# VinAIResearch/GeoFormer

Measured on NVIDIA B200. Metric: geodesic maps/sec, higher is better.
Workload: dtype f32

## Files before the change

### geoformer_b200/_capi.py

```python
import ctypes
import os
import threading

import torch

_HERE = os.path.dirname(os.path.abspath(__file__))
LIB_PATH = os.environ.get("GF_LIB") or os.path.join(_HERE, "libgeoformer_b200.so")

_lib = None
_lock = threading.Lock()

c_int, c_float, c_size_t, c_void_p, c_int64 = ctypes.c_int, ctypes.c_float, ctypes.c_size_t, ctypes.c_void_p, ctypes.c_int64

_P = c_void_p
SIGNATURES = {
    "gf_last_error": (ctypes.c_char_p, []),
    "gf_version": (c_int, []),
    "gf_launch_count": (c_int64, []),
    "gf_reset_launch_count": (None, []),
    "gf_set_stage_events": (c_int, [_P, c_int]),
    "gf_event_create": (c_void_p, []),
    "gf_event_destroy": (None, [_P]),
    "gf_event_elapsed_ms": (c_float, [_P, _P]),
    "gf_fps_workspace_bytes": (c_size_t, [c_int, c_int, c_int]),
    "gf_furthest_point_sampling": (c_int, [_P, c_int, c_int, c_int, _P, _P, c_size_t, _P]),
    "gf_gather_points": (c_int, [_P, _P, c_int, c_int, c_int, c_int, _P, _P]),
    "gf_gather_points_grad": (c_int, [_P, _P, c_int, c_int, c_int, c_int, _P, _P]),
    "gf_ball_query": (c_int, [_P, _P, c_int, c_int, c_int, c_float, c_int, _P, _P]),
    "gf_group_points": (c_int, [_P, _P, c_int, c_int, c_int, c_int, c_int, _P, _P]),
    "gf_group_points_grad": (c_int, [_P, _P, c_int, c_int, c_int, c_int, c_int, _P, _P]),
    "gf_three_nn": (c_int, [_P, _P, c_int, c_int, c_int, _P, _P, _P]),
    "gf_three_interpolate": (c_int, [_P, _P, _P, c_int, c_int, c_int, c_int, _P, _P]),
    "gf_three_interpolate_grad": (c_int, [_P, _P, _P, c_int, c_int, c_int, c_int, _P, _P]),
    "gf_knn_workspace_bytes": (c_size_t, [c_int, c_int, c_int, c_int]),
    "gf_knn": (c_int, [_P, c_int, _P, c_int, c_int, c_int, _P, _P, _P, c_int, _P, c_size_t, _P]),
    "gf_geodesic_workspace_bytes": (c_size_t, [c_int, c_int, c_int]),
    "gf_geodesic": (c_int, [_P, _P, c_int, c_int, c_int, _P, c_int, c_float, c_int, _P, _P, _P, _P, c_size_t, _P]),
    "gf_bias_workspace_bytes": (c_size_t, [c_int, c_int]),
    "gf_bias_decoder": (c_int, [_P, _P, _P, _P, _P, c_int, c_int, c_int, _P, _P, c_size_t, _P]),
    "gf_bias_decoder_fourier": (c_int, [_P, _P, _P, _P, _P, c_int, c_int, c_int, _P, c_int, c_int, _P, _P, _P, _P,
                                        c_size_t, _P]),
    "gf_bias_mask_head": (c_int, [_P, _P, _P, c_int, c_int, _P, _P, _P, c_size_t, _P]),
    "gf_rel_cross_attention_workspace_bytes": (c_size_t, [c_int, c_int, c_int]),
    "gf_rel_cross_attention": (c_int, [_P, _P, _P, c_int, c_int, c_int, _P, _P, _P, _P, _P, _P, _P, _P, _P, _P, c_size_t, _P]),
    "gf_rel_cross_attention_fused": (c_int, [_P, _P, _P, _P, _P, _P, _P, _P, c_int, _P, _P, c_int, c_int, c_int,
                                             _P, _P, _P, _P, _P, _P, _P, _P, _P, _P, c_size_t, _P]),
    "gf_rel_cross_attention_save": (c_int, [_P, _P, _P, c_int, c_int, c_int] + [_P] * 12 + [c_size_t, _P]),
    "gf_rel_cross_attention_fused_save": (c_int, [_P] * 8 + [c_int, _P, _P, c_int, c_int, c_int] + [_P] * 12
                                          + [c_size_t, _P]),
    "gf_rel_cross_attention_backward_workspace_bytes": (c_size_t, [c_int, c_int, c_int]),
    "gf_rel_cross_attention_backward": (c_int, [_P, _P, _P, c_int, c_int, c_int] + [_P] * 24 + [c_size_t, _P]),
    "gf_rel_cross_attention_fused_backward": (c_int, [_P] * 8 + [c_int, _P, _P, c_int, c_int, c_int] + [_P] * 23
                                              + [c_size_t, _P]),
    "gf_mask_head_workspace_bytes": (c_size_t, [c_int, c_int]),
    "gf_mask_head_logits": (c_int, [_P] * 9 + [c_int, c_int, c_int, _P, _P, c_size_t, _P]),
    "gf_mask_head_backward_workspace_bytes": (c_size_t, [c_int, c_int]),
    "gf_mask_head_logits_backward": (c_int, [_P] * 9 + [c_int, c_int, c_int] + [_P] * 7 + [c_size_t, _P]),
    "gf_group_mlp_pool": (c_int, [_P, _P, _P, _P, c_int, c_int, c_int, c_int, c_int, c_float, c_int, c_int, c_int, _P, _P,
# ... 116 lines not shown
```

### geoformer_b200/csrc/gf_guidance.cu

```cuda
#include <stdlib.h>

#include "gf_geodesic.cuh"
#include "gf_knn.cuh"

namespace gf {

constexpr int LANES = 4;
struct ForkJoin {
  cudaStream_t fps[LANES] = {}, knn[LANES] = {};
  cudaEvent_t fork = nullptr, join_fps[LANES] = {}, join_knn[LANES] = {};
  cudaStream_t aux = nullptr;
  cudaEvent_t join = nullptr;
};

static int get_fork_join(cudaStream_t user, ForkJoin **out, int lanes_needed = 1) {
  constexpr int SLOTS = 16;
  struct Entry {
    int dev;
    cudaStream_t user;
    ForkJoin fj;
    bool used;
  };
  static thread_local Entry pool[SLOTS];
  static thread_local int next_victim = 0;
// ... 124 lines not shown

extern "C" int gf_guidance_seeded(const float *xyz, int N, const int *seeds, int Q, int k, float radius, int max_step,
                                  float *geo, float *knn_dist, int32_t *knn_idx32, int64_t *stats, float *row_max,
                                  void *workspace, size_t workspace_bytes, void *stream) {
  return guidance_impl(xyz, N, Q, k, radius, max_step, const_cast<int *>(seeds), 1, geo, knn_dist, knn_idx32, stats,
                       workspace, workspace_bytes, stream, nullptr, 0, row_max);
}

extern "C" int gf_guidance_shard(const float *xyz, int N, int Q, int q0, int q1, int k, float radius, int max_step,
                                 int *seeds, float *geo_block, int64_t *stats, float *row_max_block, void *workspace,
                                 size_t workspace_bytes, void *stream) {
  return guidance_impl(xyz, N, Q, k, radius, max_step, seeds, 0, geo_block, nullptr, nullptr, stats, workspace,
                       workspace_bytes, stream, nullptr, 0, row_max_block, q0, q1);
}

extern "C" int gf_guidance_seeded_scatter(const float *xyz, int N, const int *seeds, int Q, int k, float radius,
                                          int max_step, float *geo, float *const *peer_geo, int n_peers,
                                          int64_t *stats, void *workspace, size_t workspace_bytes, void *stream) {
  return guidance_impl(xyz, N, Q, k, radius, max_step, const_cast<int *>(seeds), 1, geo, nullptr, nullptr, stats,
                       workspace, workspace_bytes, stream, peer_geo, n_peers);
}

namespace gf {
struct BatchPlan {
  size_t per_scene[GEO_BATCH_MAX * 4];
  size_t scratch, scratch_bytes, stats, total;
};
static int plan_batch_guidance(const int *Ns, int B, int Q, int k, BatchPlan *p, size_t *fps_b, size_t *knn_b,
                               size_t *edge_b) {
  size_t off = 0;
  int maxN = 1;
  for (int b = 0; b < B; ++b) {
    const int N = Ns[b];
    fps_b[b] = align256(gf_fps_workspace_bytes(1, N, Q));
    knn_b[b] = align256(knn_grid_workspace_bytes(N));
    edge_b[b] = align256(geodesic_workspace_bytes(N, k, 1));
    p->per_scene[b * 3 + 0] = off, off += fps_b[b];
    p->per_scene[b * 3 + 1] = off, off += knn_b[b];
    p->per_scene[b * 3 + 2] = off, off += edge_b[b];
    maxN = N > maxN ? N : maxN;
  }
  p->scratch = off;
  p->scratch_bytes = align256(geodesic_batch_scratch_bytes(maxN, (long long)Q * B));
  off += p->scratch_bytes;
  p->stats = off;
  off += align256(16 * (size_t)B);
  p->total = off + 1024;
  return maxN;
}
}

extern "C" size_t gf_guidance_batch_workspace_bytes(const int *Ns, int B, int Q, int k) {
  if (!Ns || B <= 0 || B > GEO_BATCH_MAX || Q <= 0 || k <= 0) return 0;
  for (int b = 0; b < B; ++b)
    if (Ns[b] <= 0) return 0;
  BatchPlan p;
  size_t f[GEO_BATCH_MAX], n[GEO_BATCH_MAX], e[GEO_BATCH_MAX];
  plan_batch_guidance(Ns, B, Q, k, &p, f, n, e);
  return p.total;
}

extern "C" int gf_guidance_batch(const float *const *xyz, const int *Ns, int B, int Q, int k, float radius,
                                 int max_step, int *const *seeds, int seeds_given, float *const *geo,
                                 float *const *row_max, int64_t *stats, void *workspace, size_t workspace_bytes,
// ... 2 lines not shown
  GF_CHECK_ARG(B >= 1 && B <= GEO_BATCH_MAX, "guidance_batch: B=%d outside [1,%d]", B, GEO_BATCH_MAX);
  GF_CHECK_ARG(Q >= 1, "guidance_batch: need Q >= 1");
  GF_CHECK_ARG(k >= 1 && k <= KNN_MAX_K, "guidance_batch: k=%d outside [1,%d]", k, KNN_MAX_K);
  for (int b = 0; b < B; ++b) {
    GF_CHECK_ARG(Ns[b] >= 1 && xyz[b] && seeds[b] && geo[b], "guidance_batch: scene %d: empty or null", b);
    GF_CHECK_ARG(geodesic_edge_format(Ns[b]) == 1,
                 "guidance_batch: scene %d has %d points, beyond the on-chip bitmaps of the batched kernel "
                 "(use gf_guidance per scene)", b, Ns[b]);
  }
  BatchPlan p;
  size_t fps_b[GEO_BATCH_MAX], knn_b[GEO_BATCH_MAX], edge_b[GEO_BATCH_MAX];
  plan_batch_guidance(Ns, B, Q, k, &p, fps_b, knn_b, edge_b);
  if (workspace == nullptr || workspace_bytes < p.total) {
    set_error("guidance_batch: workspace too small (%zu bytes given, %zu needed)", workspace_bytes, p.total);
    return GF_ERR_WORKSPACE;
  }
  cudaStream_t st = (cudaStream_t)stream;
  char *w = (char *)workspace;
  ForkJoin *fj = nullptr;
  const int lanes = B < LANES ? B : LANES;
  int rc = get_fork_join(st, &fj, lanes);
  if (rc) return rc;
  stage_mark(ST_BEGIN, st);
  GF_CUDA(cudaEventRecord(fj->fork, st));
  for (int l = 0; l < lanes; ++l) {
    if (!seeds_given) GF_CUDA(cudaStreamWaitEvent(fj->fps[l], fj->fork, 0));
    if (l > 0) GF_CUDA(cudaStreamWaitEvent(fj->knn[l], fj->fork, 0));
  }
  GeoSceneDesc desc[GEO_BATCH_MAX];
  int64_t *d_stats = stats ? (int64_t *)(w + p.stats) : nullptr;
  if (d_stats) GF_CUDA(cudaMemsetAsync(d_stats, 0, 16 * (size_t)B, st));
  if (!seeds_given)
    for (int b = 0; b < B; ++b) {
      rc = gf_furthest_point_sampling(xyz[b], 1, Ns[b], Q, seeds[b], w + p.per_scene[b * 3 + 0], fps_b[b],
                                      fj->fps[b % lanes]);
      if (rc) return rc;
    }
  for (int b = 0; b < B; ++b) {
    const int l = b % lanes;
    cudaStream_t ks = l == 0 ? st : fj->knn[l];
    KnnGridBuffers gb;
    rc = knn_grid_build(xyz[b], Ns[b], k, w + p.per_scene[b * 3 + 1], knn_b[b], ks, &gb);
    if (rc) return rc;
    KnnEdgeOut eo;
    eo.radius = radius;
    int enc = 0;
    rc = geodesic_edge_buffers(w + p.per_scene[b * 3 + 2], edge_b[b], Ns[b], k, 1, &eo.tgt, &eo.len, &eo.slot_bits,
                               &enc);
    if (rc) return rc;
    eo.rank = gb.rank;
    rc = knn_grid_query(gb, nullptr, Ns[b], k, 1, nullptr, nullptr, nullptr, ks, &eo);
    if (rc) return rc;
    desc[b].tgt = eo.tgt, desc[b].len = eo.len, desc[b].seeds = seeds[b], desc[b].geo = geo[b];
    desc[b].rank = gb.rank, desc[b].order = gb.order;
    desc[b].row_max = row_max ? row_max[b] : nullptr;
    desc[b].stats = d_stats ? d_stats + 2 * b : nullptr;
    desc[b].N = Ns[b], desc[b].Q = Q;
  }
  for (int l = 0; l < lanes; ++l) {
    if (!seeds_given) {
      GF_CUDA(cudaEventRecord(fj->join_fps[l], fj->fps[l]));
      GF_CUDA(cudaStreamWaitEvent(st, fj->join_fps[l], 0));
    }
    if (l > 0) {
      GF_CUDA(cudaEventRecord(fj->join_knn[l], fj->knn[l]));
      GF_CUDA(cudaStreamWaitEvent(st, fj->join_knn[l], 0));
    }
  }
  stage_mark(ST_KNN_DONE, st);
  rc = geodesic_batch_launch(desc, B, k, max_step, w + p.scratch, p.scratch_bytes, st);
  if (rc) return rc;
  if (stats) GF_CUDA(cudaMemcpyAsync(stats, d_stats, 16 * (size_t)B, cudaMemcpyDeviceToDevice, st));
  return GF_OK;
}

extern "C" size_t gf_guidance_host_workspace_bytes(int N, int Q, int k) {
  if (N <= 0 || Q <= 0 || k <= 0) return 0;
  return plan_guidance(N, Q, k).total + align256(sizeof(float) * (size_t)N * 3) + align256(sizeof(int) * (size_t)Q) +
         align256(sizeof(float) * (size_t)Q * N) + 1024;
}

extern "C" int gf_guidance_host(const float *xyz_host, int N, int Q, int k, float radius, int max_step,
                                int *seeds_host, float *geo_host, void *workspace, size_t workspace_bytes,
                                void *stream) {
  GF_CHECK_ARG(N >= 1 && Q >= 1, "guidance_host: need N >= 1 and Q >= 1");
  GF_CHECK_ARG(xyz_host && seeds_host && geo_host, "guidance_host: null host pointer");
  size_t need = gf_guidance_host_workspace_bytes(N, Q, k);
// ... 117 lines not shown
```

### geoformer_b200/csrc/gf_knn.cu

```cuda
#include "gf_knn.cuh"

namespace gf {

constexpr int KNN_MAX_CELLS = 1 << 22;
constexpr int KNN_PASS0_CELLS = 1 << 18;
constexpr int KNN_SCAN_BLOCKS = 512;
constexpr int KNN_MAX_DIM = 1024;

struct KnnGrid {
  float ox, oy, oz;
  float h, inv_h;
  float slack;
  int dx, dy, dz, ncells;
  uint32_t mm[6];
  unsigned long long sum_sq;
  unsigned done[2];
  unsigned pad_[2];
};
struct KnnCtl {
  KnnGrid g;
  unsigned long long scan_state[KNN_SCAN_BLOCKS];
};

__device__ void knn_plan(KnnGrid *g, int N, int pass, float tau, int cap) {
// ... 45 lines not shown
  __shared__ bool s_last;
  __threadfence();
  __syncthreads();
  if (threadIdx.x == 0) {
    const unsigned t = atomicAdd(counter, 1u);
    s_last = t == gridDim.x - 1;
    __threadfence();
  }
  __syncthreads();
  return s_last;
}

__device__ __forceinline__ int cell_coord(float v, float o, float inv_h, int dim) {
  float f = floorf((v - o) * inv_h);
  int c = (f >= 0.f) ? (f < (float)dim ? (int)f : dim - 1) : 0;
  return c;
}
__device__ __forceinline__ int cell_of(const KnnGrid &g, float x, float y, float z) {
  int cx = cell_coord(x, g.ox, g.inv_h, g.dx), cy = cell_coord(y, g.oy, g.inv_h, g.dy),
      cz = cell_coord(z, g.oz, g.inv_h, g.dz);
  return (cz * g.dy + cy) * g.dx + cx;
}

__global__ void __launch_bounds__(256) knn_bbox_kernel(const float *__restrict__ xyz, int N, KnnGrid *g, float tau,
                                                       int cap_coarse, int4 *__restrict__ zero_a, int n4_a,
                                                       int4 *__restrict__ zero_b, int n4_b) {
  const int gtid = blockIdx.x * blockDim.x + threadIdx.x, gsz = gridDim.x * blockDim.x;
  const int4 z4 = make_int4(0, 0, 0, 0);
  for (int i = gtid; i < n4_a; i += gsz) zero_a[i] = z4;
  for (int i = gtid; i < n4_b; i += gsz) zero_b[i] = z4;
  uint32_t lo[3] = {0u, 0u, 0u}, hi[3] = {0u, 0u, 0u};
  for (int i = gtid; i < N; i += gsz) {
#pragma unroll
    for (int a = 0; a < 3; ++a) {
      float v = __ldg(xyz + (size_t)i * 3 + a);
      if (v == v && fabsf(v) <= 3.0e38f) {
        uint32_t o = f2ord(v);
        lo[a] = max(lo[a], ~o);
        hi[a] = max(hi[a], o);
      }
    }
  }
#pragma unroll
  for (int a = 0; a < 3; ++a) {
    uint32_t l = __reduce_max_sync(0xffffffffu, lo[a]);
    uint32_t h = __reduce_max_sync(0xffffffffu, hi[a]);
    if ((threadIdx.x & 31) == 0) {
      if (l) atomicMax(&g->mm[a], l);
      if (h) atomicMax(&g->mm[3 + a], h);
    }
  }
  if (last_block_done(&g->done[0]) && threadIdx.x == 0) knn_plan(g, N, 0, tau, cap_coarse);
}

__global__ void __launch_bounds__(256) knn_count_kernel(const float *__restrict__ xyz, int N, KnnGrid *gp,
                                                        int *__restrict__ cell_count, int *__restrict__ cell_id,
                                                        int *__restrict__ slot_in_cell, float tau, int cap_fine) {
  const KnnGrid g = *gp;
  unsigned long long acc = 0;
  for (int i = blockIdx.x * blockDim.x + threadIdx.x; i < N; i += gridDim.x * blockDim.x) {
    float x = __ldg(xyz + (size_t)i * 3), y = __ldg(xyz + (size_t)i * 3 + 1), z = __ldg(xyz + (size_t)i * 3 + 2);
    int c = cell_of(g, x, y, z);
    int s = atomicAdd(cell_count + c, 1);
    if (cell_id) {
      cell_id[i] = c;
      slot_in_cell[i] = s;
    } else {
      acc += 2ull * (unsigned)s + 1ull;
    }
  }
  if (cell_id) return;
  for (int o = 16; o; o >>= 1) acc += __shfl_xor_sync(0xffffffffu, acc, o);
  if ((threadIdx.x & 31) == 0 && acc) atomicAdd(&gp->sum_sq, acc);
  if (last_block_done(&gp->done[1]) && threadIdx.x == 0) knn_plan(gp, N, 1, tau, cap_fine);
}

__global__ void __launch_bounds__(256) knn_scan_kernel(KnnCtl *ctl, const int *__restrict__ cnt,
                                                       int *__restrict__ start, int N) {
  const int n = ctl->g.ncells;
  const int chunk = (((n + KNN_SCAN_BLOCKS - 1) / KNN_SCAN_BLOCKS) + 3) & ~3;
  const int b0 = min(n, (int)blockIdx.x * chunk), b1 = min(n, b0 + chunk);
  __shared__ int ws[8];
  __shared__ int carry;
  const int lane = threadIdx.x & 31, warp = threadIdx.x >> 5;
  int acc = 0;
  for (int i = b0 + threadIdx.x; i < b1; i += 256) acc += cnt[i];
  for (int o = 16; o; o >>= 1) acc += __shfl_xor_sync(0xffffffffu, acc, o);
  if (lane == 0) ws[warp] = acc;
  __syncthreads();
  volatile unsigned long long *state = ctl->scan_state;
  if (threadIdx.x == 0) {
    int t = 0;
    for (int w = 0; w < 8; ++w) t += ws[w];
    state[blockIdx.x] = (1ull << 63) | (unsigned long long)(unsigned)t;
  }
  int pre = 0;
  for (int j = threadIdx.x; j < (int)blockIdx.x; j += 256) {
    unsigned long long v;
    while (!((v = state[j]) >> 63)) __nanosleep(20);
    pre += (int)(unsigned)(v & 0xffffffffull);
  }
  for (int o = 16; o; o >>= 1) pre += __shfl_xor_sync(0xffffffffu, pre, o);
  __syncthreads();
// ... 13 lines not shown
    for (int e = 0; e < 4; ++e) c[e] = (i0 + e < b1) ? cnt[i0 + e] : 0;
    int tsum = c[0] + c[1] + c[2] + c[3];
    int inc = tsum;
    for (int o = 1; o < 32; o <<= 1) {
      int t = __shfl_up_sync(0xffffffffu, inc, o);
      if (lane >= o) inc += t;
    }
    if (lane == 31) ws[warp] = inc;
    __syncthreads();
    int woff = 0;
    for (int w = 0; w < warp; ++w) woff += ws[w];
    int excl = carry + woff + inc - tsum;
#pragma unroll
    for (int e = 0; e < 4; ++e) {
      if (i0 + e < b1) start[i0 + e] = excl;
      excl += c[e];
    }
    __syncthreads();
    if (threadIdx.x == 255) carry = excl;
    __syncthreads();
  }
}

__global__ void knn_scatter_kernel(const float *__restrict__ xyz, int N, const int *__restrict__ cell_id,
                                   const int *__restrict__ slot_in_cell, const int *__restrict__ start,
                                   float4 *__restrict__ sorted, int *__restrict__ order, int *__restrict__ rank) {
  for (int i = blockIdx.x * blockDim.x + threadIdx.x; i < N; i += gridDim.x * blockDim.x) {
    int pos = start[cell_id[i]] + slot_in_cell[i];
    float x = __ldg(xyz + (size_t)i * 3), y = __ldg(xyz + (size_t)i * 3 + 1), z = __ldg(xyz + (size_t)i * 3 + 2);
    sorted[pos] = make_float4(x, y, z, __int_as_float(i));
    order[pos] = i;
    rank[i] = pos;
  }
}

template <int KT>
struct TopK {
  unsigned long long key[KT];
  __device__ __forceinline__ void init(int k) {
#pragma unroll
    for (int i = 0; i < KT; ++i) key[i] = (i < KT - k) ? 0ull : ~0ull;
  }
  __device__ __forceinline__ void offer(float d2, int index) {
    unsigned long long kk = ((unsigned long long)__float_as_uint(d2) << 32) | (unsigned)index;
    if (kk < key[KT - 1]) {
      bool below = true;
#pragma unroll
      for (int i = KT - 1; i > 0; --i) {
        const bool below_prev = kk < key[i - 1];
        key[i] = below_prev ? key[i - 1] : (below ? kk : key[i]);
// ... 55 lines not shown
        len[e] = ok ? d : 0.f;
      }
    }
    for (int e = k - 1 > 0 ? k - 1 : 0; e < KP; ++e) tgt[e] = none, len[e] = 0.f;
  }
  __device__ __forceinline__ void store(int k, bool do_sqrt, float *__restrict__ dist, long long *__restrict__ i64,
                                        int *__restrict__ i32) const {
#pragma unroll
    for (int i = 0; i < KT; ++i) {
      int j = i - (KT - k);
      if (j >= 0) {
        unsigned long long kk = key[i];
        bool missing = kk == ~0ull;
        float d2 = missing ? __int_as_float(0x7f800000) : __uint_as_float((unsigned)(kk >> 32));
        int id = missing ? -1 : (int)(unsigned)(kk & 0xffffffffu);
        if (dist) dist[j] = do_sqrt ? sqrtf(d2) : d2;
        if (i64) i64[j] = (long long)id;
        if (i32) i32[j] = id;
      }
    }
  }
};

constexpr int KNN_NB = 32;
constexpr int KNN_MIN_BLOCKS = 7;
template <int KT>
__global__ void __launch_bounds__(128, KT <= 16 ? KNN_MIN_BLOCKS : 1)
    knn_grid_query_kernel(const KnnGrid *__restrict__ gp, const float4 *__restrict__ sorted,
                          const int *__restrict__ start, const float *__restrict__ queries, int nq, int k,
                          int do_sqrt, float *__restrict__ dist, long long *__restrict__ idx64,
                          int *__restrict__ idx32, const KnnEdgeOut eo) {
  constexpr int LIST = KT + 16;
  __shared__ unsigned short hist[KNN_NB][128];
  __shared__ int list[LIST][128];
  const KnnGrid g = *gp;
  const int tid = threadIdx.x;
  const int s = blockIdx.x * blockDim.x + tid;
  if (s >= nq) return;
  if (eo.tgt && s == 0) {
    const int none = eo.rank ? (int)((((unsigned)nq >> 5) << 7) | ((unsigned)nq & 31u)) : nq;
    for (int e = 0; e < (1 << eo.slot_bits); ++e)
      eo.tgt[((size_t)nq << eo.slot_bits) + e] = none, eo.len[((size_t)nq << eo.slot_bits) + e] = 0.f;
  }
  float qx, qy, qz;
  int row;
  if (queries == nullptr) {
    float4 me = sorted[s];
    qx = me.x, qy = me.y, qz = me.z;
    row = __float_as_int(me.w);
  } else {
    qx = __ldg(queries + (size_t)s * 3), qy = __ldg(queries + (size_t)s * 3 + 1), qz = __ldg(queries + (size_t)s * 3 + 2);
    row = s;
  }
  const int cx = cell_coord(qx, g.ox, g.inv_h, g.dx), cy = cell_coord(qy, g.oy, g.inv_h, g.dy),
            cz = cell_coord(qz, g.oz, g.inv_h, g.dz);
  TopK<KT> top;
  top.init(k);
  auto offer_run = [&](int p, int p1) {
    for (; p + 4 <= p1; p += 4) {
      const float4 c0 = __ldg(sorted + p), c1 = __ldg(sorted + p + 1), c2 = __ldg(sorted + p + 2),
// ... 108 lines not shown
            xa = max(xl, 0), xb = min(xr, g.dx - 1);
          } else {
            xa = xb = sgi == 0 ? xl : xr;
            if (xa < 0 || xa >= g.dx) continue;
          }
          if (xa > xb) continue;
          offer_run(__ldg(start + rowbase + xa), __ldg(start + rowbase + xb + 1));
        }
      }
      if (shells_done(R)) break;
    }
  }
  if (dist || idx64 || idx32)
    top.store(k, do_sqrt != 0, dist ? dist + (size_t)row * k : nullptr, idx64 ? idx64 + (size_t)row * k : nullptr,
              idx32 ? idx32 + (size_t)row * k : nullptr);
  if (eo.tgt) {
    const size_t er = (size_t)(eo.rank ? s : row) << eo.slot_bits;
    top.store_edges(k, eo.radius, nq, eo.slot_bits, eo.rank, eo.tgt + er, eo.len + er);
  }
}

constexpr int KNN_PEND = 8;
template <int KT>
__global__ void __launch_bounds__(128, 1)
    knn_grid_query_sync_kernel(const KnnGrid *__restrict__ gp, const float4 *__restrict__ sorted,
                               const int *__restrict__ start, const float *__restrict__ queries, int nq, int k,
                               int do_sqrt, float *__restrict__ dist, long long *__restrict__ idx64,
                               int *__restrict__ idx32, const KnnEdgeOut eo) {
  __shared__ unsigned long long pend[KNN_PEND][128];
  constexpr unsigned FULL = 0xffffffffu;
  const KnnGrid g = *gp;
  const int tid = threadIdx.x;
  const int s = blockIdx.x * blockDim.x + tid;
  const bool live = s < nq;
  if (eo.tgt && s == 0) {
    const int none = eo.rank ? (int)((((unsigned)nq >> 5) << 7) | ((unsigned)nq & 31u)) : nq;
    for (int e = 0; e < (1 << eo.slot_bits); ++e)
      eo.tgt[((size_t)nq << eo.slot_bits) + e] = none, eo.len[((size_t)nq << eo.slot_bits) + e] = 0.f;
  }
  float qx = 0.f, qy = 0.f, qz = 0.f;
  int row = 0;
  if (live) {
    if (queries == nullptr) {
      float4 me = sorted[s];
      qx = me.x, qy = me.y, qz = me.z;
      row = __float_as_int(me.w);
    } else {
      qx = __ldg(queries + (size_t)s * 3), qy = __ldg(queries + (size_t)s * 3 + 1), qz = __ldg(queries + (size_t)s * 3 + 2);
      row = s;
    }
  }
  const int cx = cell_coord(qx, g.ox, g.inv_h, g.dx), cy = cell_coord(qy, g.oy, g.inv_h, g.dy),
            cz = cell_coord(qz, g.oz, g.inv_h, g.dz);
  TopK<KT> top;
  top.init(k);
  int npend = 0;
// ... 113 lines not shown

static int knn_cap_fine(int N) {
  long long c = 8ll * N;
  if (c < (1 << 18)) c = 1 << 18;
  if (c > KNN_MAX_CELLS) c = KNN_MAX_CELLS;
  return (int)c;
}
static int knn_cap_coarse(int N) {
  int c = N < 4096 ? 4096 : N;
  return c > KNN_PASS0_CELLS ? KNN_PASS0_CELLS : c;
}

size_t knn_grid_workspace_bytes(int N) {
  size_t b = 0;
  b += align256(sizeof(KnnCtl));
  b += align256(sizeof(int) * (size_t)knn_cap_coarse(N));
  b += align256(sizeof(int) * (size_t)(knn_cap_fine(N) + 4)) * 2;
  b += align256(sizeof(int) * (size_t)N) * 4;
  b += align256(sizeof(float4) * (size_t)N);
  return b + 1024;
}

template <int KT>
static void launch_grid_query(const KnnGrid *g, const float4 *sorted, const int *start, const float *queries, int nq,
                              int k, int do_sqrt, float *dist, long long *i64, int *i32, const KnnEdgeOut &eo,
                              cudaStream_t st) {
  if constexpr (KT > 32)
    knn_grid_query_sync_kernel<KT><<<(nq + 127) / 128, 128, 0, st>>>(g, sorted, start, queries, nq, k, do_sqrt, dist, i64,
                                                                     i32, eo);
  else
    knn_grid_query_kernel<KT><<<(nq + 127) / 128, 128, 0, st>>>(g, sorted, start, queries, nq, k, do_sqrt, dist, i64, i32,
                                                                eo);
}
template <int KT>
static void launch_brute(const float *xyz, int N, const float *queries, int nq, int k, int do_sqrt, float *dist,
                         long long *i64, int *i32, cudaStream_t st) {
  knn_brute_kernel<KT><<<(nq + 127) / 128, 128, 0, st>>>(xyz, N, queries, nq, k, do_sqrt, dist, i64, i32);
}

int knn_grid_build(const float *xyz, int N, int k, void *workspace, size_t workspace_bytes, cudaStream_t st,
                   KnnGridBuffers *out) {
  const int cap_fine = knn_cap_fine(N), cap_coarse = knn_cap_coarse(N);
  Arena a(workspace, workspace_bytes);
  KnnCtl *ctl = a.take<KnnCtl>(1);
  KnnGrid *g = &ctl->g;
  int *coarse_count = a.take<int>(cap_coarse);
  int *cell_count = a.take<int>(cap_fine + 4);
  int *cell_start = a.take<int>(cap_fine + 4);
  int *cell_id = a.take<int>(N);
  int *slot = a.take<int>(N);
  int *order = a.take<int>(N);
  int *rank = a.take<int>(N);
  float4 *sorted = a.take<float4>(N);
  if (!a.ok) {
    set_error("knn: workspace too small (%zu bytes given, %zu needed)", workspace_bytes, knn_grid_workspace_bytes(N));
    return GF_ERR_WORKSPACE;
  }
  const int nb = num_sms() * 8;
  const float tau_mul = k > 32 ? 0.2f : 0.45f;
  const float tau = fmaxf(2.f, tau_mul * (float)k);
  const int npt = min(nb, (N + 255) / 256);
  GF_CUDA(cudaMemsetAsync(ctl, 0, sizeof(KnnCtl), st));
  knn_bbox_kernel<<<nb, 256, 0, st>>>(xyz, N, g, tau, cap_coarse, (int4 *)coarse_count, (cap_coarse + 3) / 4,
                                      (int4 *)cell_count, (cap_fine + 4) / 4);
  GF_LAUNCHED();
  knn_count_kernel<<<npt, 256, 0, st>>>(xyz, N, g, coarse_count, nullptr, nullptr, tau, cap_fine);
  GF_LAUNCHED();
  knn_count_kernel<<<npt, 256, 0, st>>>(xyz, N, g, cell_count, cell_id, slot, tau, cap_fine);
  GF_LAUNCHED();
  knn_scan_kernel<<<KNN_SCAN_BLOCKS, 256, 0, st>>>(ctl, cell_count, cell_start, N);
  GF_LAUNCHED();
  knn_scatter_kernel<<<npt, 256, 0, st>>>(xyz, N, cell_id, slot, cell_start, sorted, order, rank);
  GF_LAUNCHED();
  out->grid = g;
  out->cell_start = cell_start;
  out->sorted = sorted;
  out->order = order;
  out->rank = rank;
  return GF_OK;
}

int knn_grid_query(const KnnGridBuffers &b, const float *queries, int nq, int k, int do_sqrt, float *dist,
                   long long *idx64, int *idx32, cudaStream_t st, const KnnEdgeOut *edges) {
  const KnnGrid *g = (const KnnGrid *)b.grid;
  KnnEdgeOut eo = {nullptr, nullptr, 0.f, 0, nullptr};
  if (edges && queries == nullptr) {
    eo = *edges;
    if (eo.rank) eo.rank = b.rank;
  }
  if (k <= 8)
    launch_grid_query<8>(g, b.sorted, b.cell_start, queries, nq, k, do_sqrt, dist, idx64, idx32, eo, st);
  else if (k <= 16)
    launch_grid_query<16>(g, b.sorted, b.cell_start, queries, nq, k, do_sqrt, dist, idx64, idx32, eo, st);
  else if (k <= 32)
    launch_grid_query<32>(g, b.sorted, b.cell_start, queries, nq, k, do_sqrt, dist, idx64, idx32, eo, st);
  else
    launch_grid_query<64>(g, b.sorted, b.cell_start, queries, nq, k, do_sqrt, dist, idx64, idx32, eo, st);
  GF_LAUNCHED();
  return GF_OK;
}

}

using namespace gf;

extern "C" size_t gf_knn_workspace_bytes(int N, int nq, int k, int algo) {
  (void)nq;
  (void)k;
  if (algo == 1 || N <= 0) return 0;
  return knn_grid_workspace_bytes(N);
}

extern "C" int gf_knn(const float *xyz, int N, const float *queries, int nq, int k, int sqrt_out, float *dist,
                      int64_t *idx64, int32_t *idx32, int algo, void *workspace, size_t workspace_bytes,
                      void *stream) {
  GF_CHECK_ARG(N >= 0 && nq >= 0, "knn: negative size");
  GF_CHECK_ARG(k >= 1 && k <= KNN_MAX_K, "knn: k=%d outside [1,%d]", k, KNN_MAX_K);
  GF_CHECK_ARG(algo == 0 || algo == 1, "knn: unknown algo %d", algo);
  cudaStream_t st = (cudaStream_t)stream;
  if (queries == nullptr) nq = N;
  if (nq == 0) return GF_OK;
  GF_CHECK_ARG(xyz || N == 0, "knn: null xyz");
  if (algo == 1 || N == 0) {
    const float *q = queries ? queries : xyz;
    if (k <= 8)
      launch_brute<8>(xyz, N, q, nq, k, sqrt_out, dist, (long long *)idx64, idx32, st);
    else if (k <= 16)
      launch_brute<16>(xyz, N, q, nq, k, sqrt_out, dist, (long long *)idx64, idx32, st);
    else if (k <= 32)
      launch_brute<32>(xyz, N, q, nq, k, sqrt_out, dist, (long long *)idx64, idx32, st);
    else
      launch_brute<64>(xyz, N, q, nq, k, sqrt_out, dist, (long long *)idx64, idx32, st);
    GF_LAUNCHED();
    return GF_OK;
  }
  KnnGridBuffers b;
  int rc = knn_grid_build(xyz, N, k, workspace, workspace_bytes, st, &b);
  if (rc) return rc;
  return knn_grid_query(b, queries, nq, k, sqrt_out, dist, (long long *)idx64, idx32, st);
}
```

### geoformer_b200/csrc/gf_knn.cuh

```cuda
#pragma once
#include "gf_common.cuh"

namespace gf {

constexpr int KNN_MAX_K = 64;

struct KnnGridBuffers {
  const void *grid;
  const int *cell_start;
  const float4 *sorted;
  const int *order;
  const int *rank;
};

struct KnnEdgeOut {
  int *tgt;
  float *len;
  float radius;
  int slot_bits;
  const int *rank;
};

size_t knn_grid_workspace_bytes(int N);
int knn_grid_build(const float *xyz, int N, int k, void *workspace, size_t workspace_bytes, cudaStream_t st,
                   KnnGridBuffers *out);
int knn_grid_query(const KnnGridBuffers &b, const float *queries, int nq, int k, int do_sqrt, float *dist,
                   long long *idx64, int *idx32, cudaStream_t st, const KnnEdgeOut *edges = nullptr);

}
```

### include/geoformer_b200.h

```cpp
#ifndef GEOFORMER_B200_H
#define GEOFORMER_B200_H

#include <stddef.h>
#include <stdint.h>

#ifdef __cplusplus
extern "C" {
#endif

#define GF_OK 0
#define GF_ERR_INVALID 1
#define GF_ERR_CUDA 2
#define GF_ERR_WORKSPACE 3

const char *gf_last_error(void);
int gf_version(void);
int64_t gf_launch_count(void);
void gf_reset_launch_count(void);

int gf_set_stage_events(void **events, int n);
void *gf_event_create(void);
void gf_event_destroy(void *event);
float gf_event_elapsed_ms(void *start, void *stop);

// ... 4 lines not shown

int gf_gather_points(const float *points, const int *idx, int B, int C, int N, int m, float *out, void *stream);
int gf_gather_points_grad(const float *grad_out, const int *idx, int B, int C, int N, int m, float *grad_points,
                          void *stream);

int gf_ball_query(const float *new_xyz, const float *xyz, int B, int N, int m, float radius, int nsample, int *idx,
                  void *stream);

int gf_group_points(const float *points, const int *idx, int B, int C, int N, int npoints, int nsample, float *out,
                    void *stream);
int gf_group_points_grad(const float *grad_out, const int *idx, int B, int C, int N, int npoints, int nsample,
                         float *grad_points, void *stream);

int gf_three_nn(const float *unknown, const float *known, int B, int n, int m, float *dist2, int *idx, void *stream);
int gf_three_interpolate(const float *points, const int *idx, const float *weight, int B, int C, int m, int n,
                         float *out, void *stream);
int gf_three_interpolate_grad(const float *grad_out, const int *idx, const float *weight, int B, int C, int n, int m,
                              float *grad_points, void *stream);


size_t gf_knn_workspace_bytes(int N, int nq, int k, int algo);
int gf_knn(const float *xyz, int N, const float *queries, int nq, int k, int sqrt_out, float *dist, int64_t *idx64,
           int32_t *idx32, int algo, void *workspace, size_t workspace_bytes, void *stream);


size_t gf_geodesic_workspace_bytes(int N, int k, int Q);
int gf_geodesic(const float *knn_dist, const void *knn_idx, int idx_is_i64, int N, int k, const int *seeds, int Q,
                float radius, int max_step, float *geo, int64_t *stats, float *row_max, void *workspace,
                size_t workspace_bytes, void *stream);


size_t gf_bias_workspace_bytes(int B, int Q);
int gf_bias_decoder(const float *const *geo_ptrs, const int *geo_ld, const int *ctx_idx, const float *query_xyz,
                    const float *ctx_xyz, int B, int Q, int C, float *out, void *workspace, size_t workspace_bytes,
                    void *stream);
int gf_bias_decoder_fourier(const float *const *geo_ptrs, const int *geo_ld, const int *ctx_idx,
                            const float *query_xyz, const float *ctx_xyz, int B, int Q, int C, const float *gauss_B,
                            int d_out, int gauss_ld, const float *pc_min, const float *pc_max, float *out,
                            void *workspace, size_t workspace_bytes, void *stream);
int gf_bias_mask_head(const float *geo, const float *coords, const float *seed_xyz, int Q, int N,
                      const float *row_max, float *out, void *workspace, size_t workspace_bytes, void *stream);

size_t gf_rel_cross_attention_workspace_bytes(int Q, int C, int B);
int gf_rel_cross_attention(const float *tgt2, const float *memory, const float *relative_pos, int Q, int C, int B,
                           const float *w1, const float *b1, const float *w2, const float *b2, const float *wv,
                           const float *bv, const float *wo, const float *bo, float *out, void *workspace,
// ... 113 lines not shown
```

Before: 1.004 million.

## Batch KNN grid build and query across scenes into single kernel launches

Moves scene count into blockIdx.y for the grid build kernels and packs all scenes' query blocks into one launch using __grid_constant__ descriptor arrays. When the batch exceeds the lane count, the per-lane fork/join streams for KNN are skipped and everything runs on the main stream. The goal is to replace many small per-scene launches and cross-stream event syncs with a handful of wide launches. In exchange, each scene gets a share of the block budget, a large kernel parameter struct, and a linear scene lookup per block. A new public gf_knn_batch entry point is also added.

```diff
diff --git a/geoformer_b200/_capi.py b/geoformer_b200/_capi.py
--- a/geoformer_b200/_capi.py
+++ b/geoformer_b200/_capi.py
@@ -34,6 +34,8 @@
     "gf_three_interpolate_grad": (c_int, [_P, _P, _P, c_int, c_int, c_int, c_int, _P, _P]),
     "gf_knn_workspace_bytes": (c_size_t, [c_int, c_int, c_int, c_int]),
     "gf_knn": (c_int, [_P, c_int, _P, c_int, c_int, c_int, _P, _P, _P, c_int, _P, c_size_t, _P]),
+    "gf_knn_batch_workspace_bytes": (c_size_t, [_P, c_int]),
+    "gf_knn_batch": (c_int, [_P, _P, c_int, c_int, c_int, _P, _P, _P, c_size_t, _P]),
     "gf_geodesic_workspace_bytes": (c_size_t, [c_int, c_int, c_int]),
     "gf_geodesic": (c_int, [_P, _P, c_int, c_int, c_int, _P, c_int, c_float, c_int, _P, _P, _P, _P, c_size_t, _P]),
     "gf_bias_workspace_bytes": (c_size_t, [c_int, c_int]),
diff --git a/geoformer_b200/csrc/gf_guidance.cu b/geoformer_b200/csrc/gf_guidance.cu
--- a/geoformer_b200/csrc/gf_guidance.cu
+++ b/geoformer_b200/csrc/gf_guidance.cu
@@ -170,9 +170,10 @@
 }
 
 namespace gf {
+static_assert(KNN_BATCH_MAX == GEO_BATCH_MAX, "one batched call builds and queries all its scenes' graphs at once");
 struct BatchPlan {
   size_t per_scene[GEO_BATCH_MAX * 4];
-  size_t scratch, scratch_bytes, stats, total;
+  size_t knn_ctl, scratch, scratch_bytes, stats, total;
 };
 static int plan_batch_guidance(const int *Ns, int B, int Q, int k, BatchPlan *p, size_t *fps_b, size_t *knn_b,
                                size_t *edge_b) {
@@ -188,6 +189,8 @@
     p->per_scene[b * 3 + 2] = off, off += edge_b[b];
     maxN = N > maxN ? N : maxN;
   }
+  p->knn_ctl = off;
+  off += align256(knn_ctl_block_bytes(B));
   p->scratch = off;
   p->scratch_bytes = align256(geodesic_batch_scratch_bytes(maxN, (long long)Q * B));
   off += p->scratch_bytes;
@@ -236,10 +239,11 @@
   int rc = get_fork_join(st, &fj, lanes);
   if (rc) return rc;
   stage_mark(ST_BEGIN, st);
+  const bool batched = B > LANES;
   GF_CUDA(cudaEventRecord(fj->fork, st));
   for (int l = 0; l < lanes; ++l) {
     if (!seeds_given) GF_CUDA(cudaStreamWaitEvent(fj->fps[l], fj->fork, 0));
-    if (l > 0) GF_CUDA(cudaStreamWaitEvent(fj->knn[l], fj->fork, 0));
+    if (l > 0 && !batched) GF_CUDA(cudaStreamWaitEvent(fj->knn[l], fj->fork, 0));
   }
   GeoSceneDesc desc[GEO_BATCH_MAX];
   int64_t *d_stats = stats ? (int64_t *)(w + p.stats) : nullptr;
@@ -250,33 +254,49 @@
                                       fj->fps[b % lanes]);
       if (rc) return rc;
     }
+  KnnBuildScene ks[GEO_BATCH_MAX];
+  KnnGridBuffers gb[GEO_BATCH_MAX];
+  KnnEdgeOut eo[GEO_BATCH_MAX];
+  KnnQueryJob jobs[GEO_BATCH_MAX];
+  for (int b = 0; b < B; ++b) ks[b] = {xyz[b], Ns[b], w + p.per_scene[b * 3 + 1], knn_b[b]};
+  if (batched) {
+    rc = knn_grid_build_batch(ks, B, k, w + p.knn_ctl, st, gb);
+    if (rc) return rc;
+  }
   for (int b = 0; b < B; ++b) {
     const int l = b % lanes;
-    cudaStream_t ks = l == 0 ? st : fj->knn[l];
-    KnnGridBuffers gb;
-    rc = knn_grid_build(xyz[b], Ns[b], k, w + p.per_scene[b * 3 + 1], knn_b[b], ks, &gb);
-    if (rc) return rc;
-    KnnEdgeOut eo;
-    eo.radius = radius;
+    cudaStream_t kst = l == 0 ? st : fj->knn[l];
+    if (!batched) {
+      rc = knn_grid_build_batch(&ks[b], 1, k, nullptr, kst, &gb[b]);
+      if (rc) return rc;
+    }
+    eo[b].radius = radius;
     int enc = 0;
-    rc = geodesic_edge_buffers(w + p.per_scene[b * 3 + 2], edge_b[b], Ns[b], k, 1, &eo.tgt, &eo.len, &eo.slot_bits,
-                               &enc);
-    if (rc) return rc;
-    eo.rank = gb.rank;
-    rc = knn_grid_query(gb, nullptr, Ns[b], k, 1, nullptr, nullptr, nullptr, ks, &eo);
-    if (rc) return rc;
-    desc[b].tgt = eo.tgt, desc[b].len = eo.len, desc[b].seeds = seeds[b], desc[b].geo = geo[b];
-    desc[b].rank = gb.rank, desc[b].order = gb.order;
+    rc = geodesic_edge_buffers(w + p.per_scene[b * 3 + 2], edge_b[b], Ns[b], k, 1, &eo[b].tgt, &eo[b].len,
+                               &eo[b].slot_bits, &enc);
+    if (rc) return rc;
+    eo[b].rank = gb[b].rank;
+    jobs[b] = {gb[b], nullptr, Ns[b], nullptr, nullptr, nullptr, &eo[b]};
+    if (!batched) {
+      rc = knn_grid_query_batch(&jobs[b], 1, k, 1, kst);
+      if (rc) return rc;
+    }
+    desc[b].tgt = eo[b].tgt, desc[b].len = eo[b].len, desc[b].seeds = seeds[b], desc[b].geo = geo[b];
+    desc[b].rank = gb[b].rank, desc[b].order = gb[b].order;
     desc[b].row_max = row_max ? row_max[b] : nullptr;
     desc[b].stats = d_stats ? d_stats + 2 * b : nullptr;
     desc[b].N = Ns[b], desc[b].Q = Q;
+  }
+  if (batched) {
+    rc = knn_grid_query_batch(jobs, B, k, 1, st);
+    if (rc) return rc;
   }
   for (int l = 0; l < lanes; ++l) {
     if (!seeds_given) {
       GF_CUDA(cudaEventRecord(fj->join_fps[l], fj->fps[l]));
       GF_CUDA(cudaStreamWaitEvent(st, fj->join_fps[l], 0));
     }
-    if (l > 0) {
+    if (l > 0 && !batched) {
       GF_CUDA(cudaEventRecord(fj->join_knn[l], fj->knn[l]));
       GF_CUDA(cudaStreamWaitEvent(st, fj->join_knn[l], 0));
     }
diff --git a/geoformer_b200/csrc/gf_knn.cu b/geoformer_b200/csrc/gf_knn.cu
--- a/geoformer_b200/csrc/gf_knn.cu
+++ b/geoformer_b200/csrc/gf_knn.cu
@@ -91,9 +91,25 @@
   return (cz * g.dy + cy) * g.dx + cx;
 }
 
-__global__ void __launch_bounds__(256) knn_bbox_kernel(const float *__restrict__ xyz, int N, KnnGrid *g, float tau,
-                                                       int cap_coarse, int4 *__restrict__ zero_a, int n4_a,
-                                                       int4 *__restrict__ zero_b, int n4_b) {
+struct KnnBuildDesc {
+  const float *xyz;
+  KnnCtl *ctl;
+  int *coarse_count, *cell_count, *cell_start, *cell_id, *slot, *order, *rank;
+  float4 *sorted;
+  int N, cap_coarse, cap_fine;
+};
+struct KnnBuildArgs {
+  KnnBuildDesc s[KNN_BATCH_MAX];
+  float tau;
+};
+
+__global__ void __launch_bounds__(256) knn_bbox_kernel(const __grid_constant__ KnnBuildArgs ba) {
+  const KnnBuildDesc &d = ba.s[blockIdx.y];
+  const float *__restrict__ xyz = d.xyz;
+  const int N = d.N;
+  KnnGrid *g = &d.ctl->g;
+  int4 *__restrict__ zero_a = (int4 *)d.coarse_count, *__restrict__ zero_b = (int4 *)d.cell_count;
+  const int n4_a = (d.cap_coarse + 3) / 4, n4_b = (d.cap_fine + 4) / 4;
   const int gtid = blockIdx.x * blockDim.x + threadIdx.x, gsz = gridDim.x * blockDim.x;
   const int4 z4 = make_int4(0, 0, 0, 0);
   for (int i = gtid; i < n4_a; i += gsz) zero_a[i] = z4;
@@ -119,12 +135,17 @@
       if (h) atomicMax(&g->mm[3 + a], h);
     }
   }
-  if (last_block_done(&g->done[0]) && threadIdx.x == 0) knn_plan(g, N, 0, tau, cap_coarse);
-}
-
-__global__ void __launch_bounds__(256) knn_count_kernel(const float *__restrict__ xyz, int N, KnnGrid *gp,
-                                                        int *__restrict__ cell_count, int *__restrict__ cell_id,
-                                                        int *__restrict__ slot_in_cell, float tau, int cap_fine) {
+  if (last_block_done(&g->done[0]) && threadIdx.x == 0) knn_plan(g, N, 0, ba.tau, d.cap_coarse);
+}
+
+__global__ void __launch_bounds__(256) knn_count_kernel(const __grid_constant__ KnnBuildArgs ba, int fine) {
+  const KnnBuildDesc &d = ba.s[blockIdx.y];
+  const float *__restrict__ xyz = d.xyz;
+  const int N = d.N;
+  KnnGrid *gp = &d.ctl->g;
+  int *__restrict__ cell_count = fine ? d.cell_count : d.coarse_count;
+  int *__restrict__ cell_id = fine ? d.cell_id : nullptr;
+  int *__restrict__ slot_in_cell = d.slot;
   const KnnGrid g = *gp;
   unsigned long long acc = 0;
   for (int i = blockIdx.x * blockDim.x + threadIdx.x; i < N; i += gridDim.x * blockDim.x) {
@@ -141,13 +162,17 @@
   if (cell_id) return;
   for (int o = 16; o; o >>= 1) acc += __shfl_xor_sync(0xffffffffu, acc, o);
   if ((threadIdx.x & 31) == 0 && acc) atomicAdd(&gp->sum_sq, acc);
-  if (last_block_done(&gp->done[1]) && threadIdx.x == 0) knn_plan(gp, N, 1, tau, cap_fine);
-}
-
-__global__ void __launch_bounds__(256) knn_scan_kernel(KnnCtl *ctl, const int *__restrict__ cnt,
-                                                       int *__restrict__ start, int N) {
+  if (last_block_done(&gp->done[1]) && threadIdx.x == 0) knn_plan(gp, N, 1, ba.tau, d.cap_fine);
+}
+
+__global__ void __launch_bounds__(256) knn_scan_kernel(const __grid_constant__ KnnBuildArgs ba) {
+  const KnnBuildDesc &d = ba.s[blockIdx.y];
+  KnnCtl *ctl = d.ctl;
+  const int *__restrict__ cnt = d.cell_count;
+  int *__restrict__ start = d.cell_start;
+  const int N = d.N;
   const int n = ctl->g.ncells;
-  const int chunk = (((n + KNN_SCAN_BLOCKS - 1) / KNN_SCAN_BLOCKS) + 3) & ~3;
+  const int chunk = (((n + (int)gridDim.x - 1) / (int)gridDim.x) + 3) & ~3;
   const int b0 = min(n, (int)blockIdx.x * chunk), b1 = min(n, b0 + chunk);
   __shared__ int ws[8];
   __shared__ int carry;
@@ -207,10 +232,13 @@
   }
 }
 
-__global__ void knn_scatter_kernel(const float *__restrict__ xyz, int N, const int *__restrict__ cell_id,
-                                   const int *__restrict__ slot_in_cell, const int *__restrict__ start,
-                                   float4 *__restrict__ sorted, int *__restrict__ order, int *__restrict__ rank) {
-  for (int i = blockIdx.x * blockDim.x + threadIdx.x; i < N; i += gridDim.x * blockDim.x) {
+__global__ void __launch_bounds__(256) knn_scatter_kernel(const __grid_constant__ KnnBuildArgs ba) {
+  const KnnBuildDesc &d = ba.s[blockIdx.y];
+  const float *__restrict__ xyz = d.xyz;
+  const int *__restrict__ cell_id = d.cell_id, *__restrict__ slot_in_cell = d.slot, *__restrict__ start = d.cell_start;
+  float4 *__restrict__ sorted = d.sorted;
+  int *__restrict__ order = d.order, *__restrict__ rank = d.rank;
+  for (int i = blockIdx.x * blockDim.x + threadIdx.x; i < d.N; i += gridDim.x * blockDim.x) {
     int pos = start[cell_id[i]] + slot_in_cell[i];
     float x = __ldg(xyz + (size_t)i * 3), y = __ldg(xyz + (size_t)i * 3 + 1), z = __ldg(xyz + (size_t)i * 3 + 2);
     sorted[pos] = make_float4(x, y, z, __int_as_float(i));
@@ -312,20 +340,47 @@
   }
 };
 
+struct KnnQueryDesc {
+  const KnnGrid *grid;
+  const float4 *sorted;
+  const int *start;
+  const float *queries;
+  float *dist;
+  long long *idx64;
+  int *idx32;
+  KnnEdgeOut eo;
+  int nq, block0;
+};
+struct KnnQueryArgs {
+  KnnQueryDesc s[KNN_BATCH_MAX];
+  int B, k, do_sqrt;
+};
+#define KNN_QUERY_SCENE(a, PTR)                                                                       \
+  int sc_ = 0;                                                                                        \
+  while (sc_ + 1 < (a).B && (int)blockIdx.x >= (a).s[sc_ + 1].block0) ++sc_;                          \
+  const KnnQueryDesc &d = (a).s[sc_];                                                                 \
+  const KnnGrid *PTR gp = d.grid;                                                                     \
+  const float4 *PTR sorted = d.sorted;                                                                \
+  const int *PTR start = d.start;                                                                     \
+  const float *PTR queries = d.queries;                                                               \
+  float *PTR dist = d.dist;                                                                           \
+  long long *PTR idx64 = d.idx64;                                                                     \
+  int *PTR idx32 = d.idx32;                                                                           \
+  const KnnEdgeOut &eo = d.eo;                                                                        \
+  const int nq = d.nq, k = (a).k, do_sqrt = (a).do_sqrt
+
 constexpr int KNN_NB = 32;
 constexpr int KNN_MIN_BLOCKS = 7;
 template <int KT>
 __global__ void __launch_bounds__(128, KT <= 16 ? KNN_MIN_BLOCKS : 1)
-    knn_grid_query_kernel(const KnnGrid *__restrict__ gp, const float4 *__restrict__ sorted,
-                          const int *__restrict__ start, const float *__restrict__ queries, int nq, int k,
-                          int do_sqrt, float *__restrict__ dist, long long *__restrict__ idx64,
-                          int *__restrict__ idx32, const KnnEdgeOut eo) {
+    knn_grid_query_kernel(const __grid_constant__ KnnQueryArgs a) {
   constexpr int LIST = KT + 16;
   __shared__ unsigned short hist[KNN_NB][128];
   __shared__ int list[LIST][128];
+  KNN_QUERY_SCENE(a, const &);
   const KnnGrid g = *gp;
   const int tid = threadIdx.x;
-  const int s = blockIdx.x * blockDim.x + tid;
+  const int s = (blockIdx.x - d.block0) * blockDim.x + tid;
   if (s >= nq) return;
   if (eo.tgt && s == 0) {
     const int none = eo.rank ? (int)((((unsigned)nq >> 5) << 7) | ((unsigned)nq & 31u)) : nq;
@@ -480,16 +535,13 @@
 
 constexpr int KNN_PEND = 8;
 template <int KT>
-__global__ void __launch_bounds__(128, 1)
-    knn_grid_query_sync_kernel(const KnnGrid *__restrict__ gp, const float4 *__restrict__ sorted,
-                               const int *__restrict__ start, const float *__restrict__ queries, int nq, int k,
-                               int do_sqrt, float *__restrict__ dist, long long *__restrict__ idx64,
-                               int *__restrict__ idx32, const KnnEdgeOut eo) {
+__global__ void __launch_bounds__(128, 1) knn_grid_query_sync_kernel(const __grid_constant__ KnnQueryArgs a) {
   __shared__ unsigned long long pend[KNN_PEND][128];
   constexpr unsigned FULL = 0xffffffffu;
+  KNN_QUERY_SCENE(a, __restrict__);
   const KnnGrid g = *gp;
   const int tid = threadIdx.x;
-  const int s = blockIdx.x * blockDim.x + tid;
+  const int s = (blockIdx.x - d.block0) * blockDim.x + tid;
   const bool live = s < nq;
   if (eo.tgt && s == 0) {
     const int none = eo.rank ? (int)((((unsigned)nq >> 5) << 7) | ((unsigned)nq & 31u)) : nq;
@@ -649,15 +701,11 @@
 }
 
 template <int KT>
-static void launch_grid_query(const KnnGrid *g, const float4 *sorted, const int *start, const float *queries, int nq,
-                              int k, int do_sqrt, float *dist, long long *i64, int *i32, const KnnEdgeOut &eo,
-                              cudaStream_t st) {
+static void launch_grid_query(const KnnQueryArgs &a, int blocks, cudaStream_t st) {
   if constexpr (KT > 32)
-    knn_grid_query_sync_kernel<KT><<<(nq + 127) / 128, 128, 0, st>>>(g, sorted, start, queries, nq, k, do_sqrt, dist, i64,
-                                                                     i32, eo);
+    knn_grid_query_sync_kernel<KT><<<blocks, 128, 0, st>>>(a);
   else
-    knn_grid_query_kernel<KT><<<(nq + 127) / 128, 128, 0, st>>>(g, sorted, start, queries, nq, k, do_sqrt, dist, i64, i32,
-                                                                eo);
+    knn_grid_query_kernel<KT><<<blocks, 128, 0, st>>>(a);
 }
 template <int KT>
 static void launch_brute(const float *xyz, int N, const float *queries, int nq, int k, int do_sqrt, float *dist,
@@ -665,66 +713,114 @@
   knn_brute_kernel<KT><<<(nq + 127) / 128, 128, 0, st>>>(xyz, N, queries, nq, k, do_sqrt, dist, i64, i32);
 }
 
+size_t knn_ctl_block_bytes(int B) { return align256(sizeof(KnnCtl)) * (size_t)(B > 0 ? B : 0); }
+
+int knn_grid_build_batch(const KnnBuildScene *scenes, int B, int k, void *ctl_block, cudaStream_t st,
+                         KnnGridBuffers *out) {
+  if (B < 1 || B > KNN_BATCH_MAX || (ctl_block == nullptr && B != 1)) {
+    set_error("knn: batched build of %d scenes (1..%d, control blocks %s)", B, KNN_BATCH_MAX,
+              ctl_block ? "given" : "missing");
+    return GF_ERR_INVALID;
+  }
+  KnnBuildArgs a;
+  int maxN = 1;
+  for (int b = 0; b < B; ++b) {
+    const int N = scenes[b].N;
+    KnnBuildDesc &d = a.s[b];
+    d.xyz = scenes[b].xyz;
+    d.N = N;
+    d.cap_fine = knn_cap_fine(N), d.cap_coarse = knn_cap_coarse(N);
+    Arena ar(scenes[b].workspace, scenes[b].workspace_bytes);
+    KnnCtl *own = ar.take<KnnCtl>(1);
+    d.ctl = ctl_block ? (KnnCtl *)((char *)ctl_block + align256(sizeof(KnnCtl)) * b) : own;
+    d.coarse_count = ar.take<int>(d.cap_coarse);
+    d.cell_count = ar.take<int>(d.cap_fine + 4);
+    d.cell_start = ar.take<int>(d.cap_fine + 4);
+    d.cell_id = ar.take<int>(N);
+    d.slot = ar.take<int>(N);
+    d.order = ar.take<int>(N);
+    d.rank = ar.take<int>(N);
+    d.sorted = ar.take<float4>(N);
+    if (!ar.ok) {
+      set_error("knn: workspace of scene %d too small (%zu bytes given, %zu needed)", b, scenes[b].workspace_bytes,
+                knn_grid_workspace_bytes(N));
+      return GF_ERR_WORKSPACE;
+    }
+    maxN = N > maxN ? N : maxN;
+    out[b].grid = &d.ctl->g;
+    out[b].cell_start = d.cell_start;
+    out[b].sorted = d.sorted;
+    out[b].order = d.order;
+    out[b].rank = d.rank;
+  }
+  const int nb = num_sms() * 8;
+  const int per_scene = nb / B > 1 ? nb / B : 1;
+  const int npt = min(per_scene, (maxN + 255) / 256);
+  const int nscan = min(per_scene, KNN_SCAN_BLOCKS);
+  const float tau_mul = k > 32 ? 0.2f : 0.45f;
+  a.tau = fmaxf(2.f, tau_mul * (float)k);
+  GF_CUDA(cudaMemsetAsync(a.s[0].ctl, 0, ctl_block ? knn_ctl_block_bytes(B) : sizeof(KnnCtl), st));
+  knn_bbox_kernel<<<dim3(per_scene, B), 256, 0, st>>>(a);
+  GF_LAUNCHED();
+  knn_count_kernel<<<dim3(npt, B), 256, 0, st>>>(a, 0);
+  GF_LAUNCHED();
+  knn_count_kernel<<<dim3(npt, B), 256, 0, st>>>(a, 1);
+  GF_LAUNCHED();
+  knn_scan_kernel<<<dim3(nscan, B), 256, 0, st>>>(a);
+  GF_LAUNCHED();
+  knn_scatter_kernel<<<dim3(npt, B), 256, 0, st>>>(a);
+  GF_LAUNCHED();
+  return GF_OK;
+}
+
 int knn_grid_build(const float *xyz, int N, int k, void *workspace, size_t workspace_bytes, cudaStream_t st,
                    KnnGridBuffers *out) {
-  const int cap_fine = knn_cap_fine(N), cap_coarse = knn_cap_coarse(N);
-  Arena a(workspace, workspace_bytes);
-  KnnCtl *ctl = a.take<KnnCtl>(1);
-  KnnGrid *g = &ctl->g;
-  int *coarse_count = a.take<int>(cap_coarse);
-  int *cell_count = a.take<int>(cap_fine + 4);
-  int *cell_start = a.take<int>(cap_fine + 4);
-  int *cell_id = a.take<int>(N);
-  int *slot = a.take<int>(N);
-  int *order = a.take<int>(N);
-  int *rank = a.take<int>(N);
-  float4 *sorted = a.take<float4>(N);
-  if (!a.ok) {
-    set_error("knn: workspace too small (%zu bytes given, %zu needed)", workspace_bytes, knn_grid_workspace_bytes(N));
-    return GF_ERR_WORKSPACE;
-  }
-  const int nb = num_sms() * 8;
-  const float tau_mul = k > 32 ? 0.2f : 0.45f;
-  const float tau = fmaxf(2.f, tau_mul * (float)k);
-  const int npt = min(nb, (N + 255) / 256);
-  GF_CUDA(cudaMemsetAsync(ctl, 0, sizeof(KnnCtl), st));
-  knn_bbox_kernel<<<nb, 256, 0, st>>>(xyz, N, g, tau, cap_coarse, (int4 *)coarse_count, (cap_coarse + 3) / 4,
-                                      (int4 *)cell_count, (cap_fine + 4) / 4);
+  const KnnBuildScene sc = {xyz, N, workspace, workspace_bytes};
+  return knn_grid_build_batch(&sc, 1, k, nullptr, st, out);
+}
+
+int knn_grid_query_batch(const KnnQueryJob *jobs, int B, int k, int do_sqrt, cudaStream_t st) {
+  if (B < 1 || B > KNN_BATCH_MAX) {
+    set_error("knn: batched query of %d scenes (1..%d)", B, KNN_BATCH_MAX);
+    return GF_ERR_INVALID;
+  }
+  KnnQueryArgs a;
+  a.B = B, a.k = k, a.do_sqrt = do_sqrt;
+  int blocks = 0;
+  for (int b = 0; b < B; ++b) {
+    const KnnQueryJob &j = jobs[b];
+    KnnQueryDesc &d = a.s[b];
+    d.grid = (const KnnGrid *)j.grid.grid;
+    d.sorted = j.grid.sorted;
+    d.start = j.grid.cell_start;
+    d.queries = j.queries;
+    d.dist = j.dist, d.idx64 = j.idx64, d.idx32 = j.idx32;
+    d.eo = {nullptr, nullptr, 0.f, 0, nullptr};
+    if (j.edges && j.queries == nullptr) {
+      d.eo = *j.edges;
+      if (d.eo.rank) d.eo.rank = j.grid.rank;
+    }
+    d.nq = j.nq;
+    d.block0 = blocks;
+    blocks += (j.nq + 127) / 128;
+  }
+  if (blocks == 0) return GF_OK;
+  if (k <= 8)
+    launch_grid_query<8>(a, blocks, st);
+  else if (k <= 16)
+    launch_grid_query<16>(a, blocks, st);
+  else if (k <= 32)
+    launch_grid_query<32>(a, blocks, st);
+  else
+    launch_grid_query<64>(a, blocks, st);
   GF_LAUNCHED();
-  knn_count_kernel<<<npt, 256, 0, st>>>(xyz, N, g, coarse_count, nullptr, nullptr, tau, cap_fine);
-  GF_LAUNCHED();
-  knn_count_kernel<<<npt, 256, 0, st>>>(xyz, N, g, cell_count, cell_id, slot, tau, cap_fine);
-  GF_LAUNCHED();
-  knn_scan_kernel<<<KNN_SCAN_BLOCKS, 256, 0, st>>>(ctl, cell_count, cell_start, N);
-  GF_LAUNCHED();
-  knn_scatter_kernel<<<npt, 256, 0, st>>>(xyz, N, cell_id, slot, cell_start, sorted, order, rank);
-  GF_LAUNCHED();
-  out->grid = g;
-  out->cell_start = cell_start;
-  out->sorted = sorted;
-  out->order = order;
-  out->rank = rank;
   return GF_OK;
 }
 
 int knn_grid_query(const KnnGridBuffers &b, const float *queries, int nq, int k, int do_sqrt, float *dist,
                    long long *idx64, int *idx32, cudaStream_t st, const KnnEdgeOut *edges) {
-  const KnnGrid *g = (const KnnGrid *)b.grid;
-  KnnEdgeOut eo = {nullptr, nullptr, 0.f, 0, nullptr};
-  if (edges && queries == nullptr) {
-    eo = *edges;
-    if (eo.rank) eo.rank = b.rank;
-  }
-  if (k <= 8)
-    launch_grid_query<8>(g, b.sorted, b.cell_start, queries, nq, k, do_sqrt, dist, idx64, idx32, eo, st);
-  else if (k <= 16)
-    launch_grid_query<16>(g, b.sorted, b.cell_start, queries, nq, k, do_sqrt, dist, idx64, idx32, eo, st);
-  else if (k <= 32)
-    launch_grid_query<32>(g, b.sorted, b.cell_start, queries, nq, k, do_sqrt, dist, idx64, idx32, eo, st);
-  else
-    launch_grid_query<64>(g, b.sorted, b.cell_start, queries, nq, k, do_sqrt, dist, idx64, idx32, eo, st);
-  GF_LAUNCHED();
-  return GF_OK;
+  const KnnQueryJob j = {b, queries, nq, dist, idx64, idx32, edges};
+  return knn_grid_query_batch(&j, 1, k, do_sqrt, st);
 }
 
 }
@@ -766,3 +862,44 @@
   if (rc) return rc;
   return knn_grid_query(b, queries, nq, k, sqrt_out, dist, (long long *)idx64, idx32, st);
 }
+
+static size_t knn_batch_layout(const int *Ns, int B, size_t *off) {
+  size_t o = align256(knn_ctl_block_bytes(B));
+  for (int b = 0; b < B; ++b) {
+    off[b] = o;
+    o += align256(knn_grid_workspace_bytes(Ns[b]));
+  }
+  return o + 1024;
+}
+
+extern "C" size_t gf_knn_batch_workspace_bytes(const int *Ns, int B) {
+  if (!Ns || B < 1 || B > KNN_BATCH_MAX) return 0;
+  for (int b = 0; b < B; ++b)
+    if (Ns[b] < 1) return 0;
+  size_t off[KNN_BATCH_MAX];
+  return knn_batch_layout(Ns, B, off);
+}
+
+extern "C" int gf_knn_batch(const float *const *xyz, const int *Ns, int B, int k, int sqrt_out, float *const *dist,
+                            int32_t *const *idx32, void *workspace, size_t workspace_bytes, void *stream) {
+  GF_CHECK_ARG(xyz && Ns && dist && idx32, "knn_batch: null pointer array");
+  GF_CHECK_ARG(B >= 1 && B <= KNN_BATCH_MAX, "knn_batch: B=%d outside [1,%d]", B, KNN_BATCH_MAX);
+  GF_CHECK_ARG(k >= 1 && k <= KNN_MAX_K, "knn_batch: k=%d outside [1,%d]", k, KNN_MAX_K);
+  for (int b = 0; b < B; ++b) GF_CHECK_ARG(Ns[b] >= 1 && xyz[b], "knn_batch: scene %d: empty or null", b);
+  size_t off[KNN_BATCH_MAX];
+  const size_t need = knn_batch_layout(Ns, B, off);
+  if (workspace == nullptr || workspace_bytes < need) {
+    set_error("knn_batch: workspace too small (%zu bytes given, %zu needed)", workspace_bytes, need);
+    return GF_ERR_WORKSPACE;
+  }
+  cudaStream_t st = (cudaStream_t)stream;
+  char *w = (char *)workspace;
+  KnnBuildScene sc[KNN_BATCH_MAX];
+  KnnGridBuffers gb[KNN_BATCH_MAX];
+  KnnQueryJob jobs[KNN_BATCH_MAX];
+  for (int b = 0; b < B; ++b) sc[b] = {xyz[b], Ns[b], w + off[b], align256(knn_grid_workspace_bytes(Ns[b]))};
+  int rc = knn_grid_build_batch(sc, B, k, w, st, gb);
+  if (rc) return rc;
+  for (int b = 0; b < B; ++b) jobs[b] = {gb[b], nullptr, Ns[b], dist[b], nullptr, idx32[b], nullptr};
+  return knn_grid_query_batch(jobs, B, k, sqrt_out, st);
+}
diff --git a/geoformer_b200/csrc/gf_knn.cuh b/geoformer_b200/csrc/gf_knn.cuh
--- a/geoformer_b200/csrc/gf_knn.cuh
+++ b/geoformer_b200/csrc/gf_knn.cuh
@@ -21,9 +21,32 @@
   const int *rank;
 };
 
+constexpr int KNN_BATCH_MAX = 32;
+
 size_t knn_grid_workspace_bytes(int N);
+size_t knn_ctl_block_bytes(int B);
+
+struct KnnBuildScene {
+  const float *xyz;
+  int N;
+  void *workspace;
+  size_t workspace_bytes;
+};
+int knn_grid_build_batch(const KnnBuildScene *scenes, int B, int k, void *ctl_block, cudaStream_t st,
+                         KnnGridBuffers *out);
 int knn_grid_build(const float *xyz, int N, int k, void *workspace, size_t workspace_bytes, cudaStream_t st,
                    KnnGridBuffers *out);
+
+struct KnnQueryJob {
+  KnnGridBuffers grid;
+  const float *queries;
+  int nq;
+  float *dist;
+  long long *idx64;
+  int *idx32;
+  const KnnEdgeOut *edges;
+};
+int knn_grid_query_batch(const KnnQueryJob *jobs, int B, int k, int do_sqrt, cudaStream_t st);
 int knn_grid_query(const KnnGridBuffers &b, const float *queries, int nq, int k, int do_sqrt, float *dist,
                    long long *idx64, int *idx32, cudaStream_t st, const KnnEdgeOut *edges = nullptr);
 
diff --git a/include/geoformer_b200.h b/include/geoformer_b200.h
--- a/include/geoformer_b200.h
+++ b/include/geoformer_b200.h
@@ -50,6 +50,10 @@
 size_t gf_knn_workspace_bytes(int N, int nq, int k, int algo);
 int gf_knn(const float *xyz, int N, const float *queries, int nq, int k, int sqrt_out, float *dist, int64_t *idx64,
            int32_t *idx32, int algo, void *workspace, size_t workspace_bytes, void *stream);
+
+size_t gf_knn_batch_workspace_bytes(const int *Ns, int B);
+int gf_knn_batch(const float *const *xyz, const int *Ns, int B, int k, int sqrt_out, float *const *dist,
+                 int32_t *const *idx32, void *workspace, size_t workspace_bytes, void *stream);
 
 
 size_t gf_geodesic_workspace_bytes(int N, int k, int Q);
```

Result: faster. 1.040 million, median of 6 (+3.6%).
